# DonggeunYu/Text2Speech

Measured on AMD Instinct MI355X. Metric: WaveGlow forward audio samples/sec (batch 8x16000 per GPU), higher is better.
Workload: dtype bf16x3 (split-bf16 products, f32 accumulate); 1 GPU; WaveGlow forward, batch 8 x 16000 samples per GPU, 12 flows, n_group 8, WN 8 layers x 512 channels (reference waveglow/config.json); per_gpu_batch=8, segment_length=16000, mode=forward, parallelism=replicas, no collective

## Files before the change

include/t2s_hip.h:

```cpp
#ifndef T2S_HIP_H
#define T2S_HIP_H
#include <stddef.h>
#ifdef __cplusplus
extern "C" {
#endif

#define T2S_OK 0
#define T2S_EINVAL (-1)
#define T2S_EHIP (-2)

#define T2S_PERM_NONE 0
#define T2S_PERM_GATE 1
#define T2S_PERM_PAIR8 2
#define T2S_ACT_NONE 0
#define T2S_ACT_RELU 1
#define T2S_ACT_TANH 2

int t2s_abi_version(void);
int t2s_operand_format(void);
int t2s_sizeof_taco_decoder(void);
int t2s_sizeof_taco_bptt(void);
const char* t2s_error_string(int code);
const char* t2s_last_hip_error(void);

// ... 21 lines not shown
                            void* stream);

int t2s_wg_audio_squeeze(float* audio, float* z, int B, int T, int n_group, int L, int unsqueeze, void* stream);

int t2s_wg_convinv(float* z, const float* W, int B, int n_group, int c_off, int n_rem, int L, void* stream);

int t2s_small_logdet_inv(const float* W, int n, float scale, float* logdet_out, float* inv_out, void* stream);

typedef struct t2s_small_mat_job { const float* W; float* logdet_out; float* inv_out; long n; } t2s_small_mat_job;
int t2s_small_logdet_inv_batch(const t2s_small_mat_job* jobs, int n_jobs, float scale, void* stream);
int t2s_small_logdet_inv_batch_host(const t2s_small_mat_job* host_jobs, int n_jobs, float scale, void* stream);

int t2s_wg_start(const float* z, const float* w, const float* bias, int B, int n_group, int c_off, int n_half, int C,
                 int L, int Lp, int halo, void* X_hi, void* X_lo, void* stream);

int t2s_wg_in_cond_gate(const void* A_hi, const void* A_lo, const float* bias, const void* X_hi, const void* X_lo,
                        const void* S_hi, const void* S_lo, void* acts_hi, void* acts_lo, int B, int C, int n_cond,
                        int taps, int dilation, int L, int Lp, int halo, int Mpad, void* stream);

int t2s_wg_res_skip(const void* A_hi, const void* A_lo, const float* bias, const void* acts_hi, const void* acts_lo,
                    void* X_hi, void* X_lo, float* skip, int B, int C, int n_res, int skip_init, int L, int Lp,
                    int halo, int Mpad, void* stream);

int t2s_wg_end_affine(const float* skip, const float* w_end, const float* b_end, float* z, float* log_s,
                      float* wn_out, int B, int n_group, int c_off, int n_half, int C, int L, int Lp, int halo, int reverse, void* stream);

typedef struct t2s_endfold_job {
    const float *w_end, *v_skip, *scale, *b_skip;
    void* fold_A;
    float* bes;
    long nj, C;
} t2s_endfold_job;
int t2s_wg_endfold_weights(const t2s_endfold_job* jobs, int n_jobs, int C, void* stream);
int t2s_wg_gate_tile_rows(int B, int C, int L);
int t2s_wg_gate_fold_slots(int B, int C, int L);
int t2s_wg_in_cond_gate_fold(const void* A_hi, const void* A_lo, const float* bias, const void* X_hi, const void* X_lo,
                             const void* S_hi, const void* S_lo, void* acts_hi, void* acts_lo, const void* fold_A,
                             float* fold_acc, int fold_init, int B, int C, int n_cond, int taps, int dilation, int L,
                             int Lp, int halo, int Mpad, void* stream);
int t2s_wg_start_window(const float* z, const float* w, const float* bias, int B, int n_group, int c_off, int n_half, int C,
                        int L, int Lp, int halo, void* X_hi, void* X_lo, int taps, int win_chunks, void* W_hi, void* W_lo,
                        void* stream);
int t2s_wg_startfold_weights(const float* v_in, const float* g_in, const float* w_start, const float* b_start, int C, int n_half,
                             int taps, int Mpad, int win_chunks, void* A_hi, void* A_lo, void* stream);
int t2s_wg_in_win_gate_fold(const void* A_hi, const void* A_lo, const float* bias, const void* W_hi, const void* W_lo,
                            const void* S_hi, const void* S_lo, void* acts_hi, void* acts_lo, const void* fold_A,
                            float* fold_acc, int fold_init, int B, int C, int n_cond, int win_chunks, int L, int Lp, int halo,
                            int Mpad, void* stream);
int t2s_wg_upsample_basis(const float* W, const float* bias, int n_mel, int ksize, int stride, int n_group, int Lp, int halo,
                          void* U_hi, void* U_lo, void* stream);
int t2s_wg_compose_cond(const float* tmp, const float* bias_in, int rows, int Mpad, int P, int K2, long ld, void* A2_hi,
                        void* A2_lo, float* bias_out, void* stream);
int t2s_wg_melwin_planes(const float* mel, int B, int n_mel, int frames, int nlag, int Fp, void* M_hi, void* M_lo, void* stream);
int t2s_wg_in_melwin_gate_fold(const void* A_hi, const void* A_lo, const void* A2_hi, const void* A2_lo, const float* bias,
                               const void* X_hi, const void* X_lo, const void* M_hi, const void* M_lo, void* acts_hi,
                               void* acts_lo, const void* fold_A, float* fold_acc, int fold_init, int B, int C, int K2,
                               int taps, int dilation, int L, int Lp, int halo, int Mpad, int P, int Fp, void* stream);
int t2s_wg_res_only(const void* A_hi, const void* A_lo, const float* bias, const void* acts_hi, const void* acts_lo,
                    void* X_hi, void* X_lo, int B, int C, int L, int Lp, int halo, int Mpad, int pair8, void* stream);
int t2s_wg_res_only_start(const void* A_hi, const void* A_lo, const float* bias, const void* acts_hi, const void* acts_lo,
                          const float* z, const float* w_start, const float* b_start, int n_group, int c_off, int n_half,
                          void* X_hi, void* X_lo, int B, int C, int L, int Lp, int halo, int Mpad, void* stream);
int t2s_wg_flow_boundary(const float* z_in, float* z_out, const float* fold_acc, int nslots, const float* bes, int n_layers,
                         const float* b_end, float* log_s, int c_off_prev, int n_half_prev, const float* W, int c_off, int n_rem,
                         int n_half, int B, int n_group, int L, int Lp, int halo, int taps, int win_chunks, void* W_hi, void* W_lo,
                         void* stream);
// ... 253 lines not shown
```

text2speech_amd/_lib.py:

```python
import ctypes
import os

HERE = os.path.dirname(os.path.abspath(__file__))
LIB_PATH = os.environ.get("T2S_LIB_PATH") or os.path.join(HERE, "libt2s_hip.so")

c_int, c_float, c_vp, c_long = ctypes.c_int, ctypes.c_float, ctypes.c_void_p, ctypes.c_long

SIGNATURES = {
    "t2s_abi_version": [],
    "t2s_operand_format": [],
    "t2s_sizeof_taco_decoder": [],
    "t2s_sizeof_taco_bptt": [],
    "t2s_error_string": [c_int],
    "t2s_last_hip_error": [],
    "t2s_plane_rows": [c_int, c_int],
    "t2s_padded_rows": [c_int],
    "t2s_pack_conv_weight": [c_vp, c_vp, c_int, c_vp, c_int, c_int, c_int, c_int, c_int, c_int, c_int, c_int, c_int,
                             c_vp, c_vp, c_vp, c_int, c_vp],
    "t2s_pack_conv_weight_table": [c_vp, c_int, c_long, c_vp],
    "t2s_weightnorm_small": [c_vp, c_vp, c_int, c_int, c_vp, c_vp],
    "t2s_wg_upsample_squeeze": [c_vp, c_vp, c_vp, c_int, c_int, c_int, c_int, c_int, c_int, c_int, c_int, c_int,
                                c_vp, c_vp, c_vp],
    "t2s_wg_audio_squeeze": [c_vp, c_vp, c_int, c_int, c_int, c_int, c_int, c_vp],
    "t2s_wg_convinv": [c_vp, c_vp, c_int, c_int, c_int, c_int, c_int, c_vp],
    "t2s_small_logdet_inv": [c_vp, c_int, c_float, c_vp, c_vp, c_vp],
    "t2s_small_logdet_inv_batch": [c_vp, c_int, c_float, c_vp],
    "t2s_small_logdet_inv_batch_host": [c_vp, c_int, c_float, c_vp],
    "t2s_wg_start": [c_vp, c_vp, c_vp, c_int, c_int, c_int, c_int, c_int, c_int, c_int, c_int, c_vp, c_vp, c_vp],
    "t2s_wg_in_cond_gate": [c_vp, c_vp, c_vp, c_vp, c_vp, c_vp, c_vp, c_vp, c_vp, c_int, c_int, c_int, c_int, c_int,
                            c_int, c_int, c_int, c_int, c_vp],
    "t2s_wg_res_skip": [c_vp, c_vp, c_vp, c_vp, c_vp, c_vp, c_vp, c_vp, c_int, c_int, c_int, c_int, c_int, c_int,
                        c_int, c_int, c_vp],
    "t2s_wg_endfold_weights": [c_vp, c_int, c_int, c_vp],
    "t2s_wg_in_cond_gate_fold": [c_vp] * 11 + [c_int] * 10 + [c_vp],
    "t2s_wg_start_window": [c_vp, c_vp, c_vp] + [c_int] * 8 + [c_vp, c_vp, c_int, c_int, c_vp, c_vp, c_vp],
    "t2s_wg_startfold_weights": [c_vp] * 4 + [c_int] * 5 + [c_vp, c_vp, c_vp],
    "t2s_wg_in_win_gate_fold": [c_vp] * 11 + [c_int] * 9 + [c_vp],
    "t2s_wg_gate_fold_slots": [c_int, c_int, c_int],
    "t2s_wg_gate_tile_rows": [c_int, c_int, c_int],
    "t2s_wg_upsample_basis": [c_vp, c_vp] + [c_int] * 6 + [c_vp, c_vp, c_vp],
    "t2s_wg_compose_cond": [c_vp, c_vp] + [c_int] * 4 + [c_long, c_vp, c_vp, c_vp, c_vp],
    "t2s_wg_melwin_planes": [c_vp] + [c_int] * 5 + [c_vp, c_vp, c_vp],
    "t2s_wg_in_melwin_gate_fold": [c_vp] * 13 + [c_int] * 12 + [c_vp],
    "t2s_wg_res_only": [c_vp] * 7 + [c_int] * 7 + [c_vp],
    "t2s_wg_res_only_start": [c_vp] * 8 + [c_int] * 3 + [c_vp, c_vp] + [c_int] * 6 + [c_vp],
    "t2s_wg_flow_boundary": [c_vp, c_vp, c_vp, c_int, c_vp, c_int, c_vp, c_vp, c_int, c_int, c_vp] + [c_int] * 10 + [c_vp, c_vp, c_vp],
    "t2s_wg_end_fold_affine": [c_vp, c_int, c_vp, c_int, c_vp, c_vp, c_vp, c_vp, c_int, c_int, c_int, c_int, c_int, c_int, c_vp],
    "t2s_wg_end_affine": [c_vp, c_vp, c_vp, c_vp, c_vp, c_vp, c_int, c_int, c_int, c_int, c_int, c_int, c_int, c_int,
                          c_int, c_vp],
    "t2s_conv_bias_act": [c_vp, c_vp, c_vp, c_vp, c_vp, c_vp, c_vp, c_vp, c_int, c_int, c_int, c_int, c_int, c_int, c_int,
                          c_int, c_int, c_int, c_int, c_vp],
    "t2s_gemv": [c_vp, c_int, c_int, c_vp, c_int, c_int, c_vp, c_int, c_long, c_vp, c_int, c_long, c_vp, c_int, c_long,
                 c_vp, c_vp, c_vp, c_long, c_long, c_int, c_int, c_int, c_vp, c_long, c_float, c_vp],
    "t2s_transpose": [c_vp, c_vp, c_int, c_int, c_vp],
    "t2s_embed_planes": [c_vp, c_vp, c_int, c_int, c_int, c_int, c_int, c_int, c_vp, c_vp, c_vp],
    "t2s_f32_to_planes": [c_vp, c_int, c_int, c_int, c_int, c_int, c_vp, c_vp, c_vp],
    "t2s_taco_parse_output": [c_vp, c_vp, c_vp, c_vp, c_int, c_int, c_int, c_vp],
    "t2s_zero_plane_rows": [c_vp, c_vp, c_vp, c_int, c_int, c_int, c_int, c_int, c_vp],
    "t2s_zero_rows_f32": [c_vp, c_vp, c_int, c_int, c_int, c_vp],
    "t2s_bn_fold": [c_vp, c_vp, c_vp, c_vp, c_vp, c_float, c_int, c_vp, c_vp, c_vp],
    "t2s_bn_train": [c_vp, c_vp, c_vp, c_float, c_int, c_vp, c_float, c_int, c_int, c_int, c_int, c_int, c_vp, c_vp, c_vp,
                     c_vp, c_vp, c_vp],
    "t2s_taco_encoder_lstm": [c_vp, c_vp, c_vp, c_vp, c_vp, c_int, c_int, c_int, c_int, c_vp, c_vp, c_vp],
    "t2s_taco_encoder_lstm_bwd": [c_vp] * 9 + [c_int] * 4 + [c_vp],
    "t2s_taco_encoder_lstm_split": [c_vp, c_vp, c_vp, c_vp, c_vp, c_int, c_int, c_int, c_int, c_vp, c_vp, c_vp, ctypes.c_uint, c_vp],
    "t2s_taco_lstm_xbuf_bytes": [c_int],
# ... 137 lines not shown
```

text2speech_amd/csrc/t2s_api.hip:

```cpp
#include "../../include/t2s_hip.h"
#include "t2s_kernels.h"
#include "t2s_api_common.h"
#include "conv_gemm_args.h"

#include <stdlib.h>
#include <string.h>

static thread_local char g_hip_err[256] = "";

extern "C" int t2s_internal_fail_hip(int ei) {
    hipError_t e = (hipError_t)ei;
    strncpy(g_hip_err, hipGetErrorString(e), sizeof(g_hip_err) - 1);
    g_hip_err[sizeof(g_hip_err) - 1] = 0;
    return T2S_EHIP;
}

extern "C" {

int t2s_abi_version(void) { return 4; }

int t2s_sizeof_taco_decoder(void) { return (int)sizeof(t2s_taco_decoder); }
int t2s_sizeof_taco_bptt(void) { return (int)sizeof(t2s_taco_bptt); }

int t2s_operand_format(void) {
#ifdef T2S_SPLIT_F16
    return 1;
#else
    return 0;
#endif
}

const char* t2s_error_string(int code) {
    switch (code) {
        case T2S_OK: return "ok";
        case T2S_EINVAL: return "invalid argument";
        case T2S_EHIP: return "HIP runtime error";
        default: return "unknown error";
    }
}
const char* t2s_last_hip_error(void) { return g_hip_err; }

int t2s_plane_rows(int L, int halo) { return cdiv(L, 256) * 256 + 2 * halo; }
int t2s_padded_rows(int rows) { return cdiv(rows, 256) * 256; }

int t2s_pack_conv_weight(const float* v, const float* g, int g_is_scale, const float* bias_in, int O, int Cin, int Kt,
                         int perm, int C_gate, int row_off, int Mpad, int koff, int Cin_pad, void* A_hi, void* A_lo,
                         float* bias_out, int bias_accumulate, void* stream) {
    if (!v || !A_hi || !A_lo || O <= 0 || Cin <= 0 || Kt <= 0) return T2S_EINVAL;
// ... 114 lines not shown
                        const void* S_hi, const void* S_lo, void* acts_hi, void* acts_lo, int B, int C, int n_cond,
                        int taps, int dilation, int L, int Lp, int halo, int Mpad, void* stream) {
    if (!planes_ok(A_hi, A_lo) || !planes_ok(X_hi, X_lo) || !planes_ok(acts_hi, acts_lo) || !bias || !al16(bias)) return T2S_EINVAL;
    if ((n_cond > 0 && !planes_ok(S_hi, S_lo)) || !gate_shape_ok(B, C, taps, dilation, L, Lp, halo, Mpad)) return T2S_EINVAL;
    ConvGemm g(A_hi, A_lo, bias);
    g.geometry(B, L, Lp, halo, Mpad);
    g.k_side(X_hi, X_lo, cdiv(C, 32), taps, dilation, S_hi, S_lo, cdiv(n_cond, 32));
    g.output(acts_hi, acts_lo, cdiv(C, 32));
    g.a.C = C;
    T2S_CHECK_HIP(g.launch(EPI_GATE, 2 * C, 256, stream));
    return T2S_OK;
}

int t2s_wg_res_skip(const void* A_hi, const void* A_lo, const float* bias, const void* acts_hi, const void* acts_lo,
                    void* X_hi, void* X_lo, float* skip, int B, int C, int n_res, int skip_init, int L, int Lp,
                    int halo, int Mpad, void* stream) {
    if (!planes_ok(A_hi, A_lo) || !planes_ok(acts_hi, acts_lo) || !bias || !al16(bias) || !skip || !al16(skip)) return T2S_EINVAL;
    if (n_res > 0 && !planes_ok(X_hi, X_lo)) return T2S_EINVAL;
    if (C <= 0 || C % 4 || (n_res != 0 && n_res != C) || !geometry_ok(B, L, Lp, halo, Mpad, n_res + C)) return T2S_EINVAL;
    ConvGemm g(A_hi, A_lo, bias);
    g.geometry(B, L, Lp, halo, Mpad);
    g.k_side(acts_hi, acts_lo, cdiv(C, 32), 1, 1);
    g.output(X_hi, X_lo, cdiv(C, 32));
    g.a.skip = skip; g.a.C = C; g.a.n_res = n_res; g.a.skip_init = skip_init;
    T2S_CHECK_HIP(g.launch(EPI_RESSKIP, n_res + C, 256, stream));
    return T2S_OK;
}

int t2s_wg_endfold_weights(const t2s_endfold_job* jobs, int n_jobs, int C, void* stream) {
    if (!jobs || n_jobs <= 0 || C <= 0 || (size_t)8 * C * sizeof(float) > 60 * 1024) return T2S_EINVAL;
    static_assert(sizeof(t2s_endfold_job) == sizeof(EndFoldJob), "t2s_endfold_job layout");
    T2S_CHECK_HIP(t2s_launch_endfold_weights((const EndFoldJob*)jobs, n_jobs, C, (hipStream_t)stream));
    return T2S_OK;
}

int t2s_wg_gate_tile_rows(int B, int C, int L) {
    if (B <= 0 || C <= 0 || L <= 0) return T2S_EINVAL;
    return gate_tile_rows(B, C, L);
}

int t2s_wg_gate_fold_slots(int B, int C, int L) {
    if (B <= 0 || C <= 0 || L <= 0) return T2S_EINVAL;
    return gate_tile_rows(B, C, L) == 128 ? 2 * cdiv(C, 64) : 2 * cdiv(C, 128);
}

int t2s_wg_in_cond_gate_fold(const void* A_hi, const void* A_lo, const float* bias, const void* X_hi, const void* X_lo,
                             const void* S_hi, const void* S_lo, void* acts_hi, void* acts_lo, const void* fold_A,
                             float* fold_acc, int fold_init, int B, int C, int n_cond, int taps, int dilation, int L,
                             int Lp, int halo, int Mpad, void* stream) {
    if (!planes_ok(A_hi, A_lo) || !planes_ok(X_hi, X_lo) || !planes_ok(acts_hi, acts_lo) || !bias || !al16(bias)) return T2S_EINVAL;
    if ((n_cond > 0 && !planes_ok(S_hi, S_lo)) || !fold_ok(fold_A, fold_acc, C)) return T2S_EINVAL;
    if (!gate_shape_ok(B, C, taps, dilation, L, Lp, halo, Mpad)) return T2S_EINVAL;
    ConvGemm g(A_hi, A_lo, bias);
    g.geometry(B, L, Lp, halo, Mpad);
    g.k_side(X_hi, X_lo, cdiv(C, 32), taps, dilation, S_hi, S_lo, cdiv(n_cond, 32));
    g.output(acts_hi, acts_lo, cdiv(C, 32));
    g.fold(fold_A, fold_acc, fold_init);
    g.a.C = C;
    T2S_CHECK_HIP(g.launch(EPI_GATE, 2 * C, gate_tile_rows(B, C, L), stream));
    return T2S_OK;
}

int t2s_wg_in_win_gate_fold(const void* A_hi, const void* A_lo, const float* bias, const void* W_hi, const void* W_lo,
                            const void* S_hi, const void* S_lo, void* acts_hi, void* acts_lo, const void* fold_A,
                            float* fold_acc, int fold_init, int B, int C, int n_cond, int win_chunks, int L, int Lp, int halo,
                            int Mpad, void* stream) {
// ... 161 lines not shown
```

text2speech_amd/csrc/t2s_kernels.h:

```cpp
#pragma once
#include <hip/hip_runtime.h>
#include <stdint.h>

typedef unsigned short u16;

enum { EPI_GATE = 0, EPI_RESSKIP = 1, EPI_BIAS_ACT = 2, EPI_GATE_BWD = 3 };
enum { ACT_NONE = 0, ACT_RELU = 1, ACT_TANH = 2 };
enum { PERM_NONE = 0, PERM_GATE = 1, PERM_PAIR8 = 2 };

struct ConvGemmArgs {
    const u16* A_hi;
    const u16* A_lo;
    const u16* X_hi;
    const u16* X_lo;
    const u16* S_hi;
    const u16* S_lo;
    const float* bias;
    u16* O_hi;
    u16* O_lo;
    float* skip;
    float* out_f32;
    int nk;
    int nk_x;
    int xc, sc, oc;
// ... 86 lines not shown
hipError_t t2s_launch_upbasis_planes(const float* W, const float* bias, int n_mel, int ksize, int stride, int n_group, int Lp,
                                     int halo, u16* U_hi, u16* U_lo, hipStream_t stream);
hipError_t t2s_launch_compose_pack(const float* tmp, const float* bias_in, int rows, int Mpad, int P, int K2, int ld, u16* A2_hi,
                                   u16* A2_lo, float* bias_out, hipStream_t stream);
hipError_t t2s_launch_melwin_planes(const float* mel, int B, int n_mel, int frames, int nlag, int Fp, u16* S_hi, u16* S_lo,
                                    hipStream_t stream);
hipError_t t2s_launch_upsample_squeeze(const float* mel, const float* W, const float* bias, int B, int n_mel,
                                       int frames, int ksize, int stride, int n_group, int L, int Lp, int halo,
                                       u16* S_hi, u16* S_lo, hipStream_t stream);
hipError_t t2s_launch_audio_squeeze(const float* audio, float* z, int B, int T, int n_group, int L, int unsqueeze,
                                    hipStream_t stream);
hipError_t t2s_launch_convinv(float* z, const float* W, int B, int n_group, int c_off, int n_rem, int L,
                              hipStream_t stream);
struct SmallMatJob { const float* W; float* logdet_out; float* inv_out; long n; };
hipError_t t2s_launch_small_logdet_batch(const SmallMatJob* jobs, int n_jobs, float scale, hipStream_t stream);
hipError_t t2s_launch_small_logdet_batch_host(const SmallMatJob* host_jobs, int n_jobs, float scale, hipStream_t stream);
hipError_t t2s_launch_small_logdet_inv(const float* W, int n, float scale, float* logdet_out, float* inv_out,
                                       hipStream_t stream);
hipError_t t2s_launch_start(const float* z, const float* w, const float* bias, int B, int n_group, int c_off,
                            int n_half, int C, int L, int Lp, int halo, u16* X_hi, u16* X_lo, hipStream_t stream,
                            int taps = 0, int nwc = 0, u16* W_hi = nullptr, u16* W_lo = nullptr);
hipError_t t2s_launch_startfold_weights(const float* v, const float* g, const float* w_start, const float* b_start, int C,
                                        int n_half, int taps, int Mpad, int nwc, u16* A_hi, u16* A_lo, hipStream_t stream);
struct EndFoldJob {
    const float* w_end;
    const float* v_skip;
    const float* scale;
    const float* b_skip;
    u16* fold_A;
    float* bes;
    long nj, C;
};
hipError_t t2s_launch_endfold_weights(const EndFoldJob* jobs, int n_jobs, int C, hipStream_t stream);
hipError_t t2s_launch_end_fold_affine(const float* fold_acc, int nslots, const float* bes, int n_layers,
                                      const float* b_end, float* z, float* log_s, float* wn_out, int B, int n_group, int c_off,
                                      int n_half, int L, int reverse, hipStream_t stream);
struct FlowBoundaryArgs {
    const float* z_in;
    float* z_out;
    const float* fold_acc;
    const float* bes;
    const float* b_end;
    float* log_s;
    const float* W;
    u16* W_hi;
    u16* W_lo;
    int nslots, n_layers, c_off_prev, nh_prev;
    int c_off, n_rem, nh;
    int G, L, Lp, halo, taps, nwc;
};
hipError_t t2s_launch_flow_boundary(const FlowBoundaryArgs& a, int B, hipStream_t stream);
int t2s_flow_boundary_max_taps();
hipError_t t2s_launch_end_affine(const float* skip, const float* w_end, const float* b_end, float* z, float* log_s,
                                 float* wn_out, int B, int n_group, int c_off, int n_half, int C, int L, int Lp, int halo,
                                 int reverse, hipStream_t stream);
```

text2speech_amd/csrc/waveglow_ops.hip:

```cpp
#include "t2s_common.h"
#include "t2s_kernels.h"

#include <string.h>

static __device__ __forceinline__ void pack_row(const float* __restrict__ vrow, const float* g, int g_is_scale, int o,
                                                 int Cin, int Kt, int perm, int C_gate, int row_off, int Mpad, int koff,
                                                 int Cin_pad, u16* A_hi, u16* A_lo, const float* bias_in,
                                                 const float* bias_in2, float* bias_out, int bias_accumulate,
                                                 float* scale_out = nullptr) {
    __shared__ float red[4];
    const int tid = threadIdx.x;
    const int n = Cin * Kt;
    float scale = 1.0f;
    if (g && g_is_scale) {
        scale = g[o];
    } else if (g) {
        float ss = 0.f;
        for (int i = tid; i < n; i += 256) {
            const float x = vrow[i];
            ss += x * x;
        }
        ss = wave_sum(ss);
        if ((tid & 63) == 0) red[tid >> 6] = ss;
        __syncthreads();
// ... 876 lines not shown
        float ss = 0.f;
        for (int i = col; i < n; i += 32) ss += vrow[i] * vrow[i];
        ss = sum16(ss);
        ss += __shfl_xor(ss, 16, 64);
        scale = g[row_ok ? o : 0] / sqrtf(ss);
    }
    __syncthreads();
    if (!row_ok) return;
    const int ncol = Kt * nw, spc = 4 / nwc;
    const int sidx = col / ncol, lc = col - sidx * ncol;
    float acc = 0.f;
    if (sidx < spc) {
        const int tap = lc / nw, j = lc - tap * nw;
#pragma unroll 8
        for (int c = 0; c < C; ++c) acc += vrow[c * Kt + tap] * s_wb[c * nw + j];
    }
    const int gate = o >= C;
    const int ch = gate ? o - C : o;
    const int p = (ch >> 7) * 256 + ((ch >> 6) & 1) * 128 + (((ch >> 4) & 3) * 2 + gate) * 16 + (ch & 15);
    for (int wc = 0; wc < nwc; ++wc) {
        u16 h, l;
        start_fold_term(acc * scale, wc * spc + sidx, true, h, l);
        A_hi[((size_t)wc * Mpad + p) * 32 + col] = h;
        A_lo[((size_t)wc * Mpad + p) * 32 + col] = l;
    }
}
hipError_t t2s_launch_startfold_weights(const float* v, const float* g, const float* w_start, const float* b_start, int C,
                                        int n_half, int taps, int Mpad, int nwc, u16* A_hi, u16* A_lo, hipStream_t stream) {
    hipLaunchKernelGGL(startfold_weights_kernel, dim3((2 * C + 7) / 8), dim3(256), (size_t)C * (n_half + 1) * sizeof(float),
                       stream, v, g, w_start, b_start, C, n_half, taps, Mpad, nwc, A_hi, A_lo);
    return hipGetLastError();
}

__global__ void end_fold_affine_kernel(const float* __restrict__ fold_acc, int nslots, const float* __restrict__ bes,
                                       int n_layers, const float* __restrict__ b_end, float* z, float* log_s, float* wn_out,
                                       int B, int G, int c_off, int nh, int L, int reverse) {
    const int t = blockIdx.x * blockDim.x + threadIdx.x;
    const int i = blockIdx.y, b = blockIdx.z;
    if (t >= L) return;
    float bb = b_end[i], ls = b_end[nh + i];
    for (int l = 0; l < n_layers; ++l) { bb += bes[l * 8 + i]; ls += bes[l * 8 + nh + i]; }
    for (int s = 0; s < nslots; ++s) {
        bb += fold_acc[(((size_t)s * B + b) * 8 + i) * L + t];
        ls += fold_acc[(((size_t)s * B + b) * 8 + nh + i) * L + t];
    }
    float* zp = z + ((size_t)b * G + c_off + nh + i) * L + t;
    const float a1 = *zp;
    *zp = reverse ? (a1 - bb) / expf(ls) : expf(ls) * a1 + bb;
    if (log_s) log_s[((size_t)b * nh + i) * L + t] = ls;
    if (wn_out) {
        wn_out[((size_t)b * 2 * nh + i) * L + t] = bb;
        wn_out[((size_t)b * 2 * nh + nh + i) * L + t] = ls;
    }
}
hipError_t t2s_launch_end_fold_affine(const float* fold_acc, int nslots, const float* bes, int n_layers,
                                      const float* b_end, float* z, float* log_s, float* wn_out, int B, int n_group, int c_off,
                                      int n_half, int L, int reverse, hipStream_t stream) {
    hipLaunchKernelGGL(end_fold_affine_kernel, dim3((L + 255) / 256, n_half, B), dim3(256), 0, stream, fold_acc, nslots, bes,
                       n_layers, b_end, z, log_s, wn_out, B, n_group, c_off, n_half, L, reverse);
    return hipGetLastError();
}

#define FB_TC 64
#define FB_EDGE 32
__global__ __launch_bounds__(256) void flow_boundary_kernel(const FlowBoundaryArgs a) {
    __shared__ float zs[16][FB_TC + FB_EDGE];
// ... 79 lines not shown
```

text2speech_amd/glow.py:

```python
import ctypes
import math

import os

import torch
import torch.nn.functional as F

from . import _lib


class _WaveGlowLossFn(torch.autograd.Function):

    @staticmethod
    def forward(ctx, sigma, n_flows, z, *rest):
        log_s = [t.detach().to(torch.float32).contiguous() for t in rest[:n_flows]]
        dets = [t.detach() for t in rest[n_flows:]]
        d0 = dets[0]
        if all(t.dtype == torch.float32 and t.dim() == 0 and t.untyped_storage().data_ptr() == d0.untyped_storage().data_ptr()
               and t.storage_offset() == d0.storage_offset() + k for k, t in enumerate(dets)):
            log_det = d0.as_strided((n_flows,), (1,))
        else:
            log_det = torch.stack([t.to(torch.float32).reshape(()) for t in dets])
        zc = z.detach().to(torch.float32).contiguous()
        dev = zc.device
# ... 131 lines not shown
        self.packed_key = None
        self.ws = {}
        self.use_fold = True
        self.grad_sync = None
        self.gemm_events = None
        self.gemm_event_stride = 1
        self._gemm_launch_no = 0

    def geom(self):
        m = self.m
        wn0 = m.WN[0]
        C, nl, ks = wn0.n_channels, wn0.n_layers, wn0.kernel_size
        n_cond = m.upsample.out_channels * m.n_group
        halo = -(-((2 ** (nl - 1)) * (ks // 2)) // 32) * 32
        g = dict(C=C, nl=nl, ks=ks, n_cond=n_cond, Cpad=-(-C // 32) * 32, Spad=-(-n_cond // 32) * 32,
                 halo=halo, Mpad1=-(-C // 128) * 256)
        g["ncol0"] = ks * (m.n_group // 2 + 1)
        g["nwc"] = 2 if 2 * g["ncol0"] <= 32 else 4
        g["nk1"] = ks * g["Cpad"] // 32 + g["Spad"] // 32
        g["nk2"] = g["Cpad"] // 32
        return g

    def start_fold_on(self):
        g = self.geom()
        if not self.use_fold or os.environ.get("T2S_START_FOLD", "1") == "0" or g["C"] % 16 or self.compose_geom() is not None:
            return False
        return g["ncol0"] <= 32 and g["Cpad"] // 32 >= g["nwc"]

    def flow_boundary_on(self):
        g = self.geom()
        return (self.start_fold_on() and os.environ.get("T2S_FLOW_BOUNDARY", "1") != "0" and g["C"] % 32 == 0 and g["nl"] >= 2
                and self.m.n_group // 2 <= 4)

    def pack_weights(self, device, force=True, flow_events=None, res_pair8=False, start_fold=False, flow_boundary=False):
        m = self.m
        res_pair8 = bool(res_pair8) and self.geom()["C"] % 32 == 0
        start_fold = bool(start_fold)
        key = tuple(p._version for p in m.parameters()) + (str(device), res_pair8, start_fold)
        flow_boundary = bool(flow_boundary) and start_fold and res_pair8
        if not force and self.packed is not None and self.packed_key == key:
            self.packed["flow_boundary"] = flow_boundary
            return self.packed
        g = self.geom()
        C, nl, ks = g["C"], g["nl"], g["ks"]
        st = _lib.current_stream()
        if self.packed is None or self.packed["device"] != device:
            flows = []
            for k in range(m.n_flows):
                n_half = m.WN[k].start.in_channels
                layers = []
                for i in range(nl):
                    rows2 = 2 * C if i < nl - 1 else C
                    Mpad2 = _lib.padded_rows(rows2)
                    layers.append(dict(
                        A1h=torch.zeros(g["nk1"], g["Mpad1"], 32, dtype=torch.bfloat16, device=device),
                        A1l=torch.zeros(g["nk1"], g["Mpad1"], 32, dtype=torch.bfloat16, device=device),
                        b1=torch.zeros(g["Mpad1"], dtype=torch.float32, device=device),
                        A2h=torch.zeros(g["nk2"], Mpad2, 32, dtype=torch.bfloat16, device=device),
                        A2l=torch.zeros(g["nk2"], Mpad2, 32, dtype=torch.bfloat16, device=device),
                        b2=torch.zeros(Mpad2, dtype=torch.float32, device=device), Mpad2=Mpad2,
                        s_in=torch.empty(2 * C, dtype=torch.float32, device=device),
                        s_cond=torch.empty(2 * C, dtype=torch.float32, device=device),
                        s_rs=torch.empty(rows2, dtype=torch.float32, device=device),
                        fold_A=torch.zeros(-(-C // 128) * 8192, dtype=torch.bfloat16, device=device)))
                flows.append(dict(layers=layers, n_half=n_half, bes=torch.zeros(nl, 8, dtype=torch.float32, device=device),
                                  w_start=torch.empty(C, n_half, dtype=torch.float32, device=device),
                                  A0h=torch.zeros(g["nwc"] + g["Spad"] // 32, g["Mpad1"], 32, dtype=torch.bfloat16, device=device),
# ... 21 lines not shown
                if i == 0 and start_fold:
                    specs[k].append((t[4], t[5], t[2], t[3], fl["A0h"], fl["A0l"], ly["b1"], 2 * C, g["n_cond"], 1, 1, C,
                                     g["Mpad1"], 32 * g["nwc"], g["Spad"], ly["s_cond"]))
                else:
                    specs[k].append((t[0], t[1], t[2], t[3], ly["A1h"], ly["A1l"], ly["b1"], 2 * C, C, ks, 1, C, g["Mpad1"], 0,
                                     g["Cpad"], ly["s_in"]))
                    specs[k].append((t[4], t[5], None, None, ly["A1h"], ly["A1l"], None, 2 * C, g["n_cond"], 1, 1, C, g["Mpad1"],
                                     ks * g["Cpad"], g["Spad"], ly["s_cond"]))
                p8 = res_pair8 and i < nl - 1
                specs[k].append((t[6], t[7], t[8], None, ly["A2h"], ly["A2l"], ly["b2"], t[6].size(0), C, 1, 2 if p8 else 0,
                                 C if p8 else 0, ly["Mpad2"], 0, g["Cpad"], ly["s_rs"]))
        ptr_key = tuple(0 if t is None else t.data_ptr() for t in srcs) + (res_pair8, start_fold)
        if self.packed.get("job_key") != ptr_key:
            rows, flow_rows, flow_jobs = [], [], []
            dp = lambda t: 0 if t is None else t.data_ptr()
            for fspecs in specs:
                row_start = 0
                flow_jobs.append((len(rows), len(fspecs)))
                for (v, gg, b1, b2, Ah, Al, bo, O, Cin, Kt, perm, Cg, Mpad, koff, Cin_pad, so) in fspecs:
                    rows.append([dp(v), dp(gg), dp(b1), dp(b2), dp(Ah), dp(Al), dp(bo), row_start,
                                 O, Cin, Kt, perm, Cg, Mpad, koff, Cin_pad, 0, 0, dp(so)])
                    row_start += -(-O // 16)
                flow_rows.append(row_start)
            self.packed["jobs"] = torch.tensor(rows, dtype=torch.int64).to(device)
            self.packed["flow_rows"] = flow_rows
            self.packed["flow_jobs"] = flow_jobs
            self.packed["job_key"] = ptr_key
        fsrc = []
        for k in range(m.n_flows):
            wn = m.WN[k]
            fl = self.packed["flows"][k]
            w_end = _f32c(wn.end.weight)
            for i in range(nl):
                vr = _f32c(_vg(wn.res_skip_layers[i])[0])
                br = _f32c(wn.res_skip_layers[i].bias)
                r0 = C if i < nl - 1 else 0
                fsrc.append((w_end, vr, br, r0, fl["layers"][i], fl["bes"], i, 2 * fl["n_half"]))
        fkey = tuple((a.data_ptr(), b.data_ptr(), c.data_ptr()) for a, b, c, *_ in fsrc)
        if self.packed.get("fold_key") != fkey:
            rows = []
            for (w_end, vr, br, r0, ly, bes, i, nj) in fsrc:
                rows.append([w_end.data_ptr(), vr.data_ptr() + 4 * r0 * C, ly["s_rs"].data_ptr() + 4 * r0,
                             br.data_ptr() + 4 * r0, ly["fold_A"].data_ptr(), bes.data_ptr() + 4 * 8 * i, nj, C])
            self.packed["fold_jobs"] = torch.tensor(rows, dtype=torch.int64).to(device)
            self.packed["fold_key"] = fkey
        jobs_ptr, fold_ptr = self.packed["jobs"].data_ptr(), self.packed["fold_jobs"].data_ptr()
        starts = []
        for k in range(m.n_flows):
            wn = m.WN[k]
            fl = self.packed["flows"][k]
            j0, nj = self.packed["flow_jobs"][k]
            _lib.call("t2s_pack_conv_weight_table", _lib.c_vp(jobs_ptr + j0 * 19 * 8), nj, self.packed["flow_rows"][k], st)
            _lib.call("t2s_wg_endfold_weights", _lib.c_vp(fold_ptr + k * nl * 8 * 8), nl, C, st)
            v, gg = _vg(wn.start)
            v, gg = _f32c(v), (None if gg is None else _f32c(gg))
            starts += [v, gg]
            _lib.call("t2s_weightnorm_small", _lib.ptr(v), _lib.ptr(gg), C, fl["n_half"], _lib.ptr(fl["w_start"]), st)
            if start_fold:
                b_start = _f32c(wn.start.bias)
                starts.append(b_start)
                _lib.call("t2s_wg_startfold_weights", _lib.ptr(in0[k][0]), _lib.ptr(in0[k][1]), _lib.ptr(fl["w_start"]),
                          _lib.ptr(b_start), C, fl["n_half"], ks, g["Mpad1"], g["nwc"], _lib.ptr(fl["A0h"]), _lib.ptr(fl["A0l"]), st)
            fl["w_inv"] = None
            if flow_events is not None:
                ev = torch.cuda.Event()
                ev.record()
                flow_events.append(ev)
        keep = srcs + [t for tup in fsrc for t in tup[:3]] + starts
        self.packed_key = key
        self.packed["res_pair8"] = res_pair8
        self.packed["start_fold"] = start_fold
        self.packed["flow_boundary"] = flow_boundary
        self._keep = keep
        return self.packed

    def compose_geom(self):
        m, g = self.m, self.geom()
        up = m.upsample
        ksz, stride, G = up.kernel_size[0], up.stride[0], m.n_group
        if os.environ.get("T2S_COND_COMPOSE") != "1" or not self.use_fold:
            return None
        if ksz % stride or stride % G or ((ksz // stride) * up.in_channels) % 32 or g["C"] % 16:
            return None
        return stride // G, ksz // stride, (ksz // stride) * up.in_channels

    def compose_cond(self, device):
        if self.packed.get("compose_key") == self.packed_key:
            return
        m, g = self.m, self.geom()
        P, nlag, K2 = self.compose_geom()
        C, nl, ks = g["C"], g["nl"], g["ks"]
        up = m.upsample
        st = _lib.current_stream()
        ncols = P * K2 + 1
        Lp_u = _lib.plane_rows(ncols, 0)
        sc = g["Spad"] // 32
        bf = dict(dtype=torch.bfloat16, device=device)
        U_h, U_l = torch.zeros(1, sc, Lp_u, 32, **bf), torch.zeros(1, sc, Lp_u, 32, **bf)
        W, bias = _f32c(up.weight), _f32c(up.bias)
        _lib.call("t2s_wg_upsample_basis", _lib.ptr(W), _lib.ptr(bias), up.in_channels, up.kernel_size[0], up.stride[0],
                  m.n_group, Lp_u, 0, _lib.ptr(U_h), _lib.ptr(U_l), st)
# ... 417 lines not shown
```

Measured before the change: 7.800 million audio samples/s.

## Fuse per-flow weight preparation into a single persistent launch

Replaces four per-flow weight-prep launches (conv weight packing, end-fold weights, start weightnorm, start fold) with one persistent kernel sized to the CU count. The blocks split end-fold slabs, start-fold items and packing groups between them. The end-fold now recomputes the res_skip weightnorm scale itself, so it no longer depends on the packing step's scale output, which lets all of the work run concurrently. It also adds a register-count query API. This cuts launch overhead and serialization in per-forward weight prep, at the cost of a more complex scheduler and a VGPR cap that may cause spills.

```diff
diff --git a/include/t2s_hip.h b/include/t2s_hip.h
--- a/include/t2s_hip.h
+++ b/include/t2s_hip.h
@@ -77,6 +77,19 @@
     long nj, C;
 } t2s_endfold_job;
 int t2s_wg_endfold_weights(const t2s_endfold_job* jobs, int n_jobs, int C, void* stream);
+typedef struct t2s_prep_fold_job {
+    const float *w_end, *v_skip, *g_skip, *b_skip;
+    void* fold_A;
+    float* bes;
+    long nj, C;
+} t2s_prep_fold_job;
+int t2s_wg_weight_prep(const t2s_pack_job* jobs, int n_jobs, long total_groups, const t2s_prep_fold_job* fold, int n_fold, int C,
+                       const float* v_start, const float* g_start, const float* b_start, int n_half, float* w_start,
+                       const float* v_in0, const float* g_in0, int taps, int Mpad, int win_chunks, void* A0_hi, void* A0_lo,
+                       void* stream);
+enum { T2S_KERNEL_WEIGHT_PREP = 0, T2S_KERNEL_LOGDET_BATCH = 1, T2S_KERNEL_GATE_GEMM = 2, T2S_KERNEL_RES_GEMM = 3,
+       T2S_KERNEL_RES_GEMM_X0 = 4 };
+int t2s_kernel_num_regs(int which);
 int t2s_wg_gate_tile_rows(int B, int C, int L);
 int t2s_wg_gate_fold_slots(int B, int C, int L);
 int t2s_wg_in_cond_gate_fold(const void* A_hi, const void* A_lo, const float* bias, const void* X_hi, const void* X_lo,
diff --git a/text2speech_amd/_lib.py b/text2speech_amd/_lib.py
--- a/text2speech_amd/_lib.py
+++ b/text2speech_amd/_lib.py
@@ -32,6 +32,9 @@
     "t2s_wg_res_skip": [c_vp, c_vp, c_vp, c_vp, c_vp, c_vp, c_vp, c_vp, c_int, c_int, c_int, c_int, c_int, c_int,
                         c_int, c_int, c_vp],
     "t2s_wg_endfold_weights": [c_vp, c_int, c_int, c_vp],
+    "t2s_wg_weight_prep": [c_vp, c_int, c_long, c_vp, c_int, c_int, c_vp, c_vp, c_vp, c_int, c_vp, c_vp, c_vp, c_int, c_int, c_int,
+                           c_vp, c_vp, c_vp],
+    "t2s_kernel_num_regs": [c_int],
     "t2s_wg_in_cond_gate_fold": [c_vp] * 11 + [c_int] * 10 + [c_vp],
     "t2s_wg_start_window": [c_vp, c_vp, c_vp] + [c_int] * 8 + [c_vp, c_vp, c_int, c_int, c_vp, c_vp, c_vp],
     "t2s_wg_startfold_weights": [c_vp] * 4 + [c_int] * 5 + [c_vp, c_vp, c_vp],
diff --git a/text2speech_amd/csrc/t2s_api.hip b/text2speech_amd/csrc/t2s_api.hip
--- a/text2speech_amd/csrc/t2s_api.hip
+++ b/text2speech_amd/csrc/t2s_api.hip
@@ -14,6 +14,9 @@
     g_hip_err[sizeof(g_hip_err) - 1] = 0;
     return T2S_EHIP;
 }
+
+template <bool PH, int EPI> __global__ void gate_gemm_pp_kernel(const ConvGemmArgs a);
+template <int EPI, int MT, bool SH, int NS, bool X0> __global__ void conv_gemm_kernel(const ConvGemmArgs a);
 
 extern "C" {
 
@@ -194,6 +197,50 @@
     static_assert(sizeof(t2s_endfold_job) == sizeof(EndFoldJob), "t2s_endfold_job layout");
     T2S_CHECK_HIP(t2s_launch_endfold_weights((const EndFoldJob*)jobs, n_jobs, C, (hipStream_t)stream));
     return T2S_OK;
+}
+
+int t2s_wg_weight_prep(const t2s_pack_job* jobs, int n_jobs, long total_groups, const t2s_prep_fold_job* fold, int n_fold, int C,
+                       const float* v_start, const float* g_start, const float* b_start, int n_half, float* w_start,
+                       const float* v_in0, const float* g_in0, int taps, int Mpad, int win_chunks, void* A0_hi, void* A0_lo,
+                       void* stream) {
+    static_assert(sizeof(t2s_pack_job) == sizeof(PackJob), "t2s_pack_job layout");
+    static_assert(sizeof(t2s_prep_fold_job) == sizeof(PrepFoldJob), "t2s_prep_fold_job layout");
+    if (!jobs || n_jobs <= 0 || total_groups <= 0 || total_groups > 0x3fffffffL || C <= 0 || n_fold < 0) return T2S_EINVAL;
+    if (n_fold > 0 && !fold) return T2S_EINVAL;
+    if (w_start && (!v_start || n_half <= 0)) return T2S_EINVAL;
+    const bool fold_start = A0_hi || A0_lo;
+    if (fold_start) {
+        if (!planes_ok(A0_hi, A0_lo) || !v_in0 || !v_start || !b_start || !win_chunks_ok(taps, n_half, win_chunks)) return T2S_EINVAL;
+        if (Mpad % 256 || Mpad < cdiv(C, 128) * 256) return T2S_EINVAL;
+    }
+    if (t2s_weight_prep_lds(C, fold_start ? n_half : 0) > 64 * 1024) return T2S_EINVAL;
+    PrepArgs a;
+    a.jobs = (const PackJob*)jobs; a.fold = (const PrepFoldJob*)fold;
+    a.v_start = v_start; a.g_start = g_start; a.b_start = b_start; a.w_start = w_start;
+    a.v_in0 = v_in0; a.g_in0 = g_in0; a.A0_hi = fold_start ? (u16*)A0_hi : nullptr; a.A0_lo = fold_start ? (u16*)A0_lo : nullptr;
+    a.n_jobs = n_jobs; a.n_groups = (int)total_groups; a.n_fold = n_fold; a.C = C; a.nh = n_half; a.Kt = taps; a.Mpad = Mpad;
+    a.nwc = win_chunks;
+    T2S_CHECK_HIP(t2s_launch_weight_prep(a, (hipStream_t)stream));
+    return T2S_OK;
+}
+
+int t2s_kernel_num_regs(int which) {
+    int n = 0;
+    hipError_t e = hipSuccess;
+    hipFuncAttributes fa;
+    switch (which) {
+        case T2S_KERNEL_WEIGHT_PREP: e = t2s_prep_kernel_num_regs(0, &n); break;
+        case T2S_KERNEL_LOGDET_BATCH: e = t2s_prep_kernel_num_regs(1, &n); break;
+        case T2S_KERNEL_GATE_GEMM:
+            e = hipFuncGetAttributes(&fa, (const void*)gate_gemm_pp_kernel<false, EPI_GATE>); n = fa.numRegs; break;
+        case T2S_KERNEL_RES_GEMM:
+            e = hipFuncGetAttributes(&fa, (const void*)conv_gemm_kernel<EPI_RESSKIP, 128, false, 2, false>); n = fa.numRegs; break;
+        case T2S_KERNEL_RES_GEMM_X0:
+            e = hipFuncGetAttributes(&fa, (const void*)conv_gemm_kernel<EPI_RESSKIP, 128, false, 2, true>); n = fa.numRegs; break;
+        default: return T2S_EINVAL;
+    }
+    if (e != hipSuccess) return t2s_internal_fail_hip((int)e);
+    return n;
 }
 
 int t2s_wg_gate_tile_rows(int B, int C, int L) {
diff --git a/text2speech_amd/csrc/t2s_kernels.h b/text2speech_amd/csrc/t2s_kernels.h
--- a/text2speech_amd/csrc/t2s_kernels.h
+++ b/text2speech_amd/csrc/t2s_kernels.h
@@ -142,6 +142,23 @@
     long nj, C;
 };
 hipError_t t2s_launch_endfold_weights(const EndFoldJob* jobs, int n_jobs, int C, hipStream_t stream);
+struct PrepFoldJob {
+    const float* w_end; const float* v_skip; const float* g_skip; const float* b_skip;
+    u16* fold_A; float* bes;
+    long nj, C;
+};
+struct PrepArgs {
+    const PackJob* jobs;
+    const PrepFoldJob* fold;
+    const float* v_start; const float* g_start; const float* b_start;
+    float* w_start;
+    const float* v_in0; const float* g_in0;
+    u16* A0_hi; u16* A0_lo;
+    int n_jobs, n_groups, n_fold, C, nh, Kt, Mpad, nwc;
+};
+size_t t2s_weight_prep_lds(int C, int n_half);
+hipError_t t2s_launch_weight_prep(const PrepArgs& a, hipStream_t stream);
+hipError_t t2s_prep_kernel_num_regs(int which, int* out);
 hipError_t t2s_launch_end_fold_affine(const float* fold_acc, int nslots, const float* bes, int n_layers,
                                       const float* b_end, float* z, float* log_s, float* wn_out, int B, int n_group, int c_off,
                                       int n_half, int L, int reverse, hipStream_t stream);
diff --git a/text2speech_amd/csrc/waveglow_ops.hip b/text2speech_amd/csrc/waveglow_ops.hip
--- a/text2speech_amd/csrc/waveglow_ops.hip
+++ b/text2speech_amd/csrc/waveglow_ops.hip
@@ -932,6 +932,294 @@
     return hipGetLastError();
 }
 
+#define PREP_VGPRS 48
+#define PREP_ATTR __attribute__((amdgpu_num_vgpr(PREP_VGPRS / 2)))
+#define PREP_END_COLS 256
+#define PREP_END_ROUNDS 6
+static __device__ __forceinline__ int prep_tid() {
+    int t = threadIdx.x;
+    asm volatile("" : "+v"(t));
+    return t;
+}
+template <int KT>
+static __device__ __forceinline__ void prep_pack_rows(const PackJob& j, int o0) {
+    const int tid = prep_tid(), r = tid >> 4, cp = tid & 15;
+    const int O = (int)j.O, Cin = (int)j.Cin, Cin_pad = (int)j.Cin_pad, koff = (int)j.koff;
+    const int o = o0 + r;
+    const bool row_ok = o < O;
+    const int n = Cin * KT;
+    const int nchunk = (Cin + 31) >> 5;
+    const float* vrow = j.v + (size_t)(row_ok ? o : 0) * n;
+    float scale = 1.0f;
+    if (j.g) {
+        if (j.g_is_scale) {
+            scale = j.g[row_ok ? o : 0];
+        } else {
+            float ss = 0.f;
+#pragma unroll 4
+            for (int cc = 0; cc < nchunk; ++cc) {
+                const int c = cc * 32 + cp * 2;
+                float x[2 * KT];
+#pragma unroll
+                for (int e = 0; e < 2 * KT; ++e) x[e] = (c + e / KT < Cin) ? vrow[c * KT + e] : 0.f;
+#pragma unroll
+                for (int e = 0; e < 2 * KT; ++e) ss += x[e] * x[e];
+            }
+            ss = sum16(ss);
+            scale = j.g[row_ok ? o : 0] / sqrtf(ss);
+        }
+    }
+    if (!row_ok) return;
+    const int p = pack_dst_row(j, o);
+    if (cp == 0) {
+        if (j.scale_out) j.scale_out[o] = scale;
+        if (j.bias_out) {
+            float bi = j.bias_in ? j.bias_in[o] : 0.f;
+            if (j.bias_in2) bi += j.bias_in2[o];
+            j.bias_out[p] = bi;
+        }
+    }
+#pragma unroll 2
+    for (int cc = 0; cc < nchunk; ++cc) {
+        const int c = cc * 32 + cp * 2;
+        float x[2 * KT];
+#pragma unroll
+        for (int e = 0; e < 2 * KT; ++e) x[e] = (c + e / KT < Cin) ? vrow[c * KT + e] : 0.f;
+#pragma unroll
+        for (int tap = 0; tap < KT; ++tap) pack_store2(j, koff + tap * Cin_pad + c, p, x[tap] * scale, x[KT + tap] * scale);
+    }
+}
+
+static __device__ __forceinline__ void prep_pack_rows_any(const PackJob& j, int o0) {
+    const int tid = prep_tid(), r = tid >> 4, cp = tid & 15;
+    const int O = (int)j.O, Cin = (int)j.Cin, Kt = (int)j.Kt, Cin_pad = (int)j.Cin_pad, koff = (int)j.koff;
+    const int o = o0 + r;
+    const bool row_ok = o < O;
+    const int n = Cin * Kt;
+    const float* vrow = j.v + (size_t)(row_ok ? o : 0) * n;
+    float scale = 1.0f;
+    if (j.g) {
+        if (j.g_is_scale) {
+            scale = j.g[row_ok ? o : 0];
+        } else {
+            float ss = 0.f;
+#pragma unroll 4
+            for (int i = cp; i < n; i += 16) ss += vrow[i] * vrow[i];
+            ss = sum16(ss);
+            scale = j.g[row_ok ? o : 0] / sqrtf(ss);
+        }
+    }
+    if (!row_ok) return;
+    const int p = pack_dst_row(j, o);
+    if (cp == 0) {
+        if (j.scale_out) j.scale_out[o] = scale;
+        if (j.bias_out) {
+            float bi = j.bias_in ? j.bias_in[o] : 0.f;
+            if (j.bias_in2) bi += j.bias_in2[o];
+            j.bias_out[p] = bi;
+        }
+    }
+    const int nchunk = (Cin + 31) >> 5;
+    for (int cc = 0; cc < nchunk; ++cc) {
+        const int c = cc * 32 + cp * 2;
+        for (int tap = 0; tap < Kt; ++tap) {
+            const float w0 = c < Cin ? vrow[c * Kt + tap] * scale : 0.f;
+            const float w1 = c + 1 < Cin ? vrow[(c + 1) * Kt + tap] * scale : 0.f;
+            pack_store2(j, koff + tap * Cin_pad + c, p, w0, w1);
+        }
+    }
+}
+
+static __device__ __forceinline__ void prep_start_table(const PrepArgs& a, float* s_wb, bool write_w) {
+    const int nh = a.nh, nw = a.nh + 1;
+    for (int c = prep_tid(); c < a.C; c += 256) {
+        float ss = 0.f;
+        for (int k = 0; k < nh; ++k) ss += a.v_start[c * nh + k] * a.v_start[c * nh + k];
+        const float s = a.g_start ? a.g_start[c] / sqrtf(ss) : 1.f;
+        for (int k = 0; k < nh; ++k) {
+            const float w = a.v_start[c * nh + k] * s;
+            if (s_wb) s_wb[c * nw + k] = w;
+            if (write_w) a.w_start[c * nh + k] = w;
+        }
+        if (s_wb) s_wb[c * nw + nh] = a.b_start[c];
+    }
+}
+
+static __device__ __forceinline__ void prep_start_item(const PrepArgs& a, int blk, const float* s_wb) {
+    const int tid = prep_tid(), r = tid >> 5, col = tid & 31;
+    const int C = a.C, Kt = a.Kt, nwc = a.nwc, nw = a.nh + 1, n = C * Kt;
+    const int o = blk * 8 + r;
+    if (o >= 2 * C) return;
+    const float* vrow = a.v_in0 + (size_t)o * n;
+    float scale = 1.0f;
+    if (a.g_in0) {
+        float ss = 0.f;
+#pragma unroll 4
+        for (int i = col; i < n; i += 32) ss += vrow[i] * vrow[i];
+        ss = sum16(ss);
+        ss += __shfl_xor(ss, 16, 64);
+        scale = a.g_in0[o] / sqrtf(ss);
+    }
+    const int ncol = Kt * nw, spc = 4 / nwc;
+    const int sidx = col / ncol, lc = col - sidx * ncol;
+    float acc = 0.f;
+    if (sidx < spc) {
+        const int tap = lc / nw, j = lc - tap * nw;
+#pragma unroll 8
+        for (int c = 0; c < C; ++c) acc += vrow[c * Kt + tap] * s_wb[c * nw + j];
+    }
+    const int gate = o >= C;
+    const int ch = gate ? o - C : o;
+    const int p = (ch >> 7) * 256 + ((ch >> 6) & 1) * 128 + (((ch >> 4) & 3) * 2 + gate) * 16 + (ch & 15);
+    for (int wc = 0; wc < nwc; ++wc) {
+        u16 h, l;
+        start_fold_term(acc * scale, wc * spc + sidx, true, h, l);
+        a.A0_hi[((size_t)wc * a.Mpad + p) * 32 + col] = h;
+        a.A0_lo[((size_t)wc * a.Mpad + p) * 32 + col] = l;
+    }
+}
+
+static __device__ __forceinline__ void prep_end_item(const PrepFoldJob& j, int slab, int C, float* smem) {
+    float* ws = smem;
+    const int tid = prep_tid(), lane = tid & 63, wave = tid >> 6;
+    const int nj = (int)j.nj;
+    {
+        const int r16 = tid >> 4, cp = tid & 15;
+        const unsigned loff = (unsigned)(r16 * C + cp * 2);
+        for (int o0 = 0; o0 < C; o0 += 16) {
+            const int o = o0 + r16;
+            const bool ok = o < C;
+            const float* vblk = j.v_skip + (size_t)o0 * C;
+            float scale = 1.0f;
+            if (j.g_skip) {
+                float ss = 0.f;
+#pragma unroll 8
+                for (int i = 0; i < C; i += 32) {
+                    const float x0 = (ok && cp * 2 + i < C) ? vblk[loff + i] : 0.f;
+                    const float x1 = (ok && cp * 2 + i + 1 < C) ? vblk[loff + i + 1] : 0.f;
+                    ss += x0 * x0;
+                    ss += x1 * x1;
+                }
+                ss = sum16(ss);
+                scale = j.g_skip[ok ? o : 0] / sqrtf(ss);
+            }
+            if (ok && cp < 8) ws[o * 8 + cp] = cp < nj ? j.w_end[(size_t)cp * C + o] * scale : 0.f;
+        }
+    }
+    __syncthreads();
+    const int wv = __builtin_amdgcn_readfirstlane(wave);
+    const int cw = slab * PREP_END_COLS + wv * 64;
+    const int c = cw + lane;
+    const bool c_ok = c < C;
+    float acc[8];
+#pragma unroll
+    for (int r = 0; r < 8; ++r) acc[r] = 0.f;
+    const float* vcol = j.v_skip + cw;
+    for (int o0 = 0; o0 < C; o0 += 5) {
+        float v[5];
+#pragma unroll
+        for (int u = 0; u < 5; ++u) v[u] = (c_ok && o0 + u < C) ? (vcol + (size_t)(o0 + u) * C)[lane] : 0.f;
+#pragma unroll
+        for (int u = 0; u < 5; ++u) {
+            const int o = o0 + u < C ? o0 + u : 0;
+            const float4 w0 = *(const float4*)(ws + o * 8), w1 = *(const float4*)(ws + o * 8 + 4);
+            acc[0] += w0.x * v[u]; acc[1] += w0.y * v[u]; acc[2] += w0.z * v[u]; acc[3] += w0.w * v[u];
+            acc[4] += w1.x * v[u]; acc[5] += w1.y * v[u]; acc[6] += w1.z * v[u]; acc[7] += w1.w * v[u];
+        }
+    }
+    if (c_ok) {
+        const int mt = c >> 7, wr = (c >> 6) & 1, pair = (c >> 5) & 1, half = (c >> 4) & 1, q = (c >> 2) & 3, reg = c & 3;
+        u16* base = j.fold_A + ((size_t)((mt * 2 + wr) * 2 + pair) * 2 * 64) * 8;
+#pragma unroll
+        for (int r = 0; r < 8; ++r) {
+            u16 h, l;
+            split_bf16(acc[r], h, l);
+            const int ln = q * 16 + r;
+            base[(size_t)ln * 8 + half * 4 + reg] = h;
+            base[(size_t)(64 + ln) * 8 + half * 4 + reg] = l;
+        }
+    }
+    if (slab == 0) {
+        float* red = smem;
+        for (int r = 0; r < 8; ++r) {
+            float s = 0.f;
+            if (r < nj)
+                for (int o = tid; o < C; o += 256) s += j.w_end[(size_t)r * C + o] * j.b_skip[o];
+            s = wave_sum(s);
+            __syncthreads();
+            if (lane == 0) red[wave] = s;
+            __syncthreads();
+            if (tid == 0) j.bes[r] = red[0] + red[1] + red[2] + red[3];
+        }
+    }
+}
+
+__global__ __launch_bounds__(256) PREP_ATTR void weight_prep_kernel(const PrepArgs a, const PackJob* __restrict__ jobs,
+                                                                             const PrepFoldJob* __restrict__ fold) {
+    extern __shared__ __attribute__((aligned(16))) float prep_smem[];
+    const int slabs = (a.C + PREP_END_COLS - 1) / PREP_END_COLS;
+    const int n_end = a.n_fold * slabs;
+    const int n_start = a.A0_hi ? (2 * a.C + 7) >> 3 : 0;
+    if (blockIdx.x == 0 && a.w_start) prep_start_table(a, nullptr, true);
+    bool have_table = false;
+    for (int it = blockIdx.x; it < n_end + n_start; it += gridDim.x) {
+        if (it < n_end) {
+            __syncthreads();
+            const PrepFoldJob j = fold[it / slabs];
+            prep_end_item(j, it % slabs, a.C, prep_smem);
+        } else {
+            if (!have_table) {
+                __syncthreads();
+                prep_start_table(a, prep_smem, false);
+                __syncthreads();
+                have_table = true;
+            }
+            prep_start_item(a, it - n_end, prep_smem);
+        }
+    }
+    const int grid = (int)gridDim.x, ne = n_end < grid ? n_end : 0, wide = grid - ne;
+    const int late = ne ? PREP_END_ROUNDS : 0;
+    for (int r = (int)blockIdx.x < ne ? late : 0;; ++r) {
+        const int blk = r < late ? r * wide + ((int)blockIdx.x - ne) : late * wide + (r - late) * grid + (int)blockIdx.x;
+        if (blk >= a.n_groups) break;
+        int lo = 0, hi = a.n_jobs - 1;
+        while (lo < hi) {
+            const int mid = (lo + hi + 1) >> 1;
+            if (jobs[mid].row_start <= blk) lo = mid; else hi = mid - 1;
+        }
+        const PackJob j = jobs[lo];
+        const int o0 = (blk - (int)j.row_start) * 16;
+        if (!((int)j.Cin & 1) && j.Kt == 3) prep_pack_rows<3>(j, o0);
+        else if (!((int)j.Cin & 1) && j.Kt == 1) prep_pack_rows<1>(j, o0);
+        else prep_pack_rows_any(j, o0);
+    }
+}
+size_t t2s_weight_prep_lds(int C, int n_half) {
+    const size_t end = (size_t)(8 * C > 16 ? 8 * C : 16) * sizeof(float), start = (size_t)C * (n_half + 1) * sizeof(float);
+    return end > start ? end : start;
+}
+hipError_t t2s_launch_weight_prep(const PrepArgs& a, hipStream_t stream) {
+    static int n_cu = 0;
+    if (!n_cu) {
+        int dev = 0, v = 0;
+        hipError_t e = hipGetDevice(&dev);
+        if (e == hipSuccess) e = hipDeviceGetAttribute(&v, hipDeviceAttributeMultiprocessorCount, dev);
+        if (e != hipSuccess) return e;
+        n_cu = v > 0 ? v : 1;
+    }
+    const int slabs = (a.C + PREP_END_COLS - 1) / PREP_END_COLS;
+    const long total = (long)a.n_fold * slabs + (a.A0_hi ? (2 * a.C + 7) / 8 : 0) + a.n_groups;
+    const int grid = (int)(total < n_cu ? (total > 0 ? total : 1) : n_cu);
+    hipLaunchKernelGGL(weight_prep_kernel, dim3(grid), dim3(256), t2s_weight_prep_lds(a.C, a.nh), stream, a, a.jobs, a.fold);
+    return hipGetLastError();
+}
+hipError_t t2s_prep_kernel_num_regs(int which, int* out) {
+    hipFuncAttributes fa;
+    hipError_t e = hipFuncGetAttributes(&fa, which == 0 ? (const void*)weight_prep_kernel : (const void*)small_logdet_batch_val_kernel);
+    if (e == hipSuccess) *out = fa.numRegs;
+    return e;
+}
+
 __global__ void end_fold_affine_kernel(const float* __restrict__ fold_acc, int nslots, const float* __restrict__ bes,
                                        int n_layers, const float* __restrict__ b_end, float* z, float* log_s, float* wn_out,
                                        int B, int G, int c_off, int nh, int L, int reverse) {
diff --git a/text2speech_amd/glow.py b/text2speech_amd/glow.py
--- a/text2speech_amd/glow.py
+++ b/text2speech_amd/glow.py
@@ -187,7 +187,8 @@
         return (self.start_fold_on() and os.environ.get("T2S_FLOW_BOUNDARY", "1") != "0" and g["C"] % 32 == 0 and g["nl"] >= 2
                 and self.m.n_group // 2 <= 4)
 
-    def pack_weights(self, device, force=True, flow_events=None, res_pair8=False, start_fold=False, flow_boundary=False):
+    def pack_weights(self, device, force=True, flow_events=None, res_pair8=False, start_fold=False, flow_boundary=False,
+                     one_launch=True):
         m = self.m
         res_pair8 = bool(res_pair8) and self.geom()["C"] % 32 == 0
         start_fold = bool(start_fold)
@@ -275,15 +276,21 @@
             fl = self.packed["flows"][k]
             w_end = _f32c(wn.end.weight)
             for i in range(nl):
-                vr = _f32c(_vg(wn.res_skip_layers[i])[0])
+                vr, gr = _vg(wn.res_skip_layers[i])
+                vr, gr = _f32c(vr), (None if gr is None else _f32c(gr))
                 br = _f32c(wn.res_skip_layers[i].bias)
                 r0 = C if i < nl - 1 else 0
-                fsrc.append((w_end, vr, br, r0, fl["layers"][i], fl["bes"], i, 2 * fl["n_half"]))
-        fkey = tuple((a.data_ptr(), b.data_ptr(), c.data_ptr()) for a, b, c, *_ in fsrc)
+                fsrc.append((w_end, vr, br, r0, fl["layers"][i], fl["bes"], i, 2 * fl["n_half"], gr))
+        fkey = tuple((a.data_ptr(), b.data_ptr(), c.data_ptr(), 0 if t[8] is None else t[8].data_ptr())
+                     for t in fsrc for a, b, c in [t[:3]]) + (bool(one_launch),)
         if self.packed.get("fold_key") != fkey:
             rows = []
-            for (w_end, vr, br, r0, ly, bes, i, nj) in fsrc:
-                rows.append([w_end.data_ptr(), vr.data_ptr() + 4 * r0 * C, ly["s_rs"].data_ptr() + 4 * r0,
+            for (w_end, vr, br, r0, ly, bes, i, nj, gr) in fsrc:
+                if one_launch:
+                    third = 0 if gr is None else gr.data_ptr() + 4 * r0
+                else:
+                    third = ly["s_rs"].data_ptr() + 4 * r0
+                rows.append([w_end.data_ptr(), vr.data_ptr() + 4 * r0 * C, third,
                              br.data_ptr() + 4 * r0, ly["fold_A"].data_ptr(), bes.data_ptr() + 4 * 8 * i, nj, C])
             self.packed["fold_jobs"] = torch.tensor(rows, dtype=torch.int64).to(device)
             self.packed["fold_key"] = fkey
@@ -293,23 +300,30 @@
             wn = m.WN[k]
             fl = self.packed["flows"][k]
             j0, nj = self.packed["flow_jobs"][k]
-            _lib.call("t2s_pack_conv_weight_table", _lib.c_vp(jobs_ptr + j0 * 19 * 8), nj, self.packed["flow_rows"][k], st)
-            _lib.call("t2s_wg_endfold_weights", _lib.c_vp(fold_ptr + k * nl * 8 * 8), nl, C, st)
             v, gg = _vg(wn.start)
             v, gg = _f32c(v), (None if gg is None else _f32c(gg))
-            starts += [v, gg]
-            _lib.call("t2s_weightnorm_small", _lib.ptr(v), _lib.ptr(gg), C, fl["n_half"], _lib.ptr(fl["w_start"]), st)
-            if start_fold:
-                b_start = _f32c(wn.start.bias)
-                starts.append(b_start)
-                _lib.call("t2s_wg_startfold_weights", _lib.ptr(in0[k][0]), _lib.ptr(in0[k][1]), _lib.ptr(fl["w_start"]),
-                          _lib.ptr(b_start), C, fl["n_half"], ks, g["Mpad1"], g["nwc"], _lib.ptr(fl["A0h"]), _lib.ptr(fl["A0l"]), st)
+            b_start = _f32c(wn.start.bias) if start_fold else None
+            starts += [v, gg, b_start]
+            if one_launch:
+                _lib.call("t2s_wg_weight_prep", _lib.c_vp(jobs_ptr + j0 * 19 * 8), nj, self.packed["flow_rows"][k],
+                          _lib.c_vp(fold_ptr + k * nl * 8 * 8), nl, C, _lib.ptr(v), _lib.ptr(gg), _lib.ptr(b_start), fl["n_half"],
+                          _lib.ptr(fl["w_start"]), _lib.ptr(in0[k][0]) if start_fold else None,
+                          _lib.ptr(in0[k][1]) if start_fold else None, ks, g["Mpad1"], g["nwc"],
+                          _lib.ptr(fl["A0h"]) if start_fold else None, _lib.ptr(fl["A0l"]) if start_fold else None, st)
+            else:
+                _lib.call("t2s_pack_conv_weight_table", _lib.c_vp(jobs_ptr + j0 * 19 * 8), nj, self.packed["flow_rows"][k], st)
+                _lib.call("t2s_wg_endfold_weights", _lib.c_vp(fold_ptr + k * nl * 8 * 8), nl, C, st)
+                _lib.call("t2s_weightnorm_small", _lib.ptr(v), _lib.ptr(gg), C, fl["n_half"], _lib.ptr(fl["w_start"]), st)
+                if start_fold:
+                    _lib.call("t2s_wg_startfold_weights", _lib.ptr(in0[k][0]), _lib.ptr(in0[k][1]), _lib.ptr(fl["w_start"]),
+                              _lib.ptr(b_start), C, fl["n_half"], ks, g["Mpad1"], g["nwc"], _lib.ptr(fl["A0h"]),
+                              _lib.ptr(fl["A0l"]), st)
             fl["w_inv"] = None
             if flow_events is not None:
                 ev = torch.cuda.Event()
                 ev.record()
                 flow_events.append(ev)
-        keep = srcs + [t for tup in fsrc for t in tup[:3]] + starts
+        keep = srcs + [t for tup in fsrc for t in tup[:3] + tup[8:]] + starts
         self.packed_key = key
         self.packed["res_pair8"] = res_pair8
         self.packed["start_fold"] = start_fold
```

Measured after the change: 7.860 million audio samples/s (median of 6 runs). About the same (+0.8%).
